# rll/rllab

Hardware: NVIDIA H100
Metric: env-steps/sec (full iteration: rollout + process_samples + VPG update) (higher is better)
Workload: dtype f32

## Files before the change

rllab_b200/csrc/update_umma32.cu:

```cuda
#include "tile_gram.cuh"
#include "umma_common.cuh"

namespace b200rl {

constexpr int V_THREADS = 128, V_TILE = 128, V_LD = V_TILE + 4;
#ifndef B200RL_V_PACKED_GRAM
#define B200RL_V_PACKED_GRAM 1
#endif

template <class N, int MODE>
struct Umma32 {
  static constexpr int O = N::O, H = 32, A = N::A;
  static_assert(N::H1 == 32 && N::H2 == 32 && O <= 24, "tensor-core 32-wide kernel: (32,32) nets, obs_dim <= 24");
  static constexpr int KX = ((O + 7) / 8) * 8;
  static constexpr int IMG = 32 * 32 * 4, IMGX = 32 * KX * 4;
  static constexpr int o_bXT = 0, o_bW1T = o_bXT + 2 * IMGX, o_bW1 = o_bW1T + 2 * IMG,
                       o_bV1T = o_bW1 + (MODE == MODE_LOSS ? 0 : 2 * IMG),
                       o_img_end = o_bV1T + (MODE == MODE_FVP ? 2 * IMG : 0);
  static constexpr int n_small = ((64 + 2 * H * A + A + 3) / 4) * 4;
  static constexpr int o_small = o_img_end, o_stage = o_small + n_small * 4;
  static constexpr int rX = 0, rH1 = rX + O, rH2 = rH1 + H, rD1 = rH2, rD2 = rH2 + H, rDM = rD2 + H, rDL = rDM + A,
                       R = (MODE == MODE_LOSS) ? 0 : rDL + A;
  static constexpr int RR = O + (MODE == MODE_FVP ? 0 : 2 * A + 1), qX = 0, qAct = O, qOm = O + A, qAdv = O + 2 * A;
  static constexpr int w_red = ((R * V_LD * 4 + 15) / 16) * 16, w_ring = w_red + 3 * 32 * 8,
                       w_bytes = w_ring + 2 * RR * V_LD * 4;
  static constexpr int o_wg = ((o_stage + 15) / 16) * 16;
  static_assert(MODE == MODE_LOSS || 2 * 64 * 16 * 8 <= R * V_LD * 4, "stage region must hold the K-half combine scratch");
  static constexpr int NWG = (MODE == MODE_LOSS || (is_grad_mode(MODE) && A == 1)) ? 3 : 2;
  static constexpr size_t bytes = (size_t)o_wg + (size_t)NWG * w_bytes;
  static_assert(bytes <= 232448, "does not fit the 227 KB of shared memory");
};

__device__ __forceinline__ void v_wg_sync(int wg) { asm volatile("bar.sync %0, 128;" ::"r"(wg + 1) : "memory"); }

template <int K, bool IS_MAX>
__device__ __forceinline__ void v_wg_reduce_store(const double (&v)[K], double* scratch, double* out, int tid, int wg) {
  const int lane = tid & 31, warp = tid >> 5;
#pragma unroll
  for (int k = 0; k < K; ++k) {
    double s = IS_MAX ? warp_max(v[k]) : warp_sum(v[k]);
    if (lane == 0) scratch[k * 32 + warp] = s;
  }
  v_wg_sync(wg);
  if (warp == 0) {
#pragma unroll
    for (int k = 0; k < K; ++k) {
      double s = lane < 4 ? scratch[k * 32 + lane] : (IS_MAX ? -1.0e300 : 0.0);
      s = IS_MAX ? warp_max(s) : warp_sum(s);
      if (lane == 0) out[k] = s;
    }
  }
  v_wg_sync(wg);
}

template <class SMT>
__device__ __forceinline__ void v_ring_load(const UpdArgs& a, float* ring, int slot, long long tile, int tid) {
  long long s = tile * V_TILE + tid;
  if (s >= a.B) s = a.B - 1;
  float* dst = ring + (size_t)slot * SMT::RR * V_LD + tid;
#pragma unroll
  for (int q = 0; q < SMT::RR; ++q) {
    const float* src = q < SMT::qAct ? a.obs + (size_t)q * a.B + s
                       : q < SMT::qOm ? a.act + (size_t)(q - SMT::qAct) * a.B + s
                       : q < SMT::qAdv ? a.old_mean + (size_t)(q - SMT::qOm) * a.B + s
                                       : a.adv + s;
    asm volatile("cp.async.ca.shared.global [%0], [%1], 4;" ::"r"(u_smem_u32(dst + q * V_LD)), "l"(src) : "memory");
  }
  asm volatile("cp.async.commit_group;" ::: "memory");
}

__device__ __forceinline__ int v_boff(int n, int k) {
  const int kp = u_kperm(k);
  return (kp & 3) * 4 + (n & 7) * 16 + (n >> 3) * 128 + (kp >> 2) * 512;
}

template <class N, int MODE>
__global__ void __launch_bounds__(V_THREADS * Umma32<N, MODE>::NWG, 1) update_umma32_kernel(UpdArgs a) {
  using SM = Umma32<N, MODE>;
  constexpr int O = N::O, H = 32, A = N::A, P = N::P, LD = V_LD, KX = SM::KX, KSX = KX / 8;
  extern __shared__ __align__(1024) unsigned char smem[];
  float* small = reinterpret_cast<float*>(smem + SM::o_small);
  float* sb0 = small, *sb1 = small + H, *sWout = small + 2 * H, *sVout = sWout + H * A;
  float* sbo = (MODE == MODE_FVP) ? sVout + H * A : sWout + H * A;
  constexpr int NWG = SM::NWG, NT = NWG * V_THREADS;
  const int gtid = threadIdx.x, wg = gtid >> 7, tid = gtid & (V_THREADS - 1), warp = tid >> 5, lane = tid & 31, t4 = lane & 3;
  unsigned char* wreg = smem + SM::o_wg + (size_t)wg * SM::w_bytes;
  float* stage = reinterpret_cast<float*>(wreg);
  double* red_scratch = reinterpret_cast<double*>(wreg + SM::w_red);
  float* ring = reinterpret_cast<float*>(wreg + SM::w_ring);

  for (int e = gtid; e < H * H; e += NT) {
    const int i = e / H, j = e % H;
    const float w = a.params[N::oW1 + e];
    const float wh = tf32_hi(w);
    *reinterpret_cast<float*>(smem + SM::o_bW1T + v_boff(j, i)) = wh;
    *reinterpret_cast<float*>(smem + SM::o_bW1T + SM::IMG + v_boff(j, i)) = w - wh;
    if constexpr (MODE != MODE_LOSS) {
      *reinterpret_cast<float*>(smem + SM::o_bW1 + v_boff(i, j)) = wh;
      *reinterpret_cast<float*>(smem + SM::o_bW1 + SM::IMG + v_boff(i, j)) = w - wh;
    }
    if constexpr (MODE == MODE_FVP) {
      const float v = (float)a.xvec[N::oW1 + e];
      const float vh = tf32_hi(v);
      *reinterpret_cast<float*>(smem + SM::o_bV1T + v_boff(j, i)) = vh;
      *reinterpret_cast<float*>(smem + SM::o_bV1T + SM::IMG + v_boff(j, i)) = v - vh;
    }
  }
  for (int e = gtid; e < KX * H; e += NT) {
    const int o = e / H, j = e % H;
    float v = 0.f;
    if (o < O) v = (MODE == MODE_FVP) ? (float)a.xvec[N::oW0 + o * H + j] : a.params[N::oW0 + o * H + j];
    const float vh = tf32_hi(v);
    *reinterpret_cast<float*>(smem + SM::o_bXT + v_boff(j, o)) = vh;
    *reinterpret_cast<float*>(smem + SM::o_bXT + SM::IMGX + v_boff(j, o)) = v - vh;
  }
  for (int e = gtid; e < H * A; e += NT) {
    sWout[e] = a.params[N::oWo + e];
    if constexpr (MODE == MODE_FVP) sVout[e] = (float)a.xvec[N::oWo + e];
  }
  for (int e = gtid; e < H; e += NT) {
    sb0[e] = (MODE == MODE_FVP) ? (float)a.xvec[N::ob0 + e] : a.params[N::ob0 + e];
    sb1[e] = (MODE == MODE_FVP) ? (float)a.xvec[N::ob1 + e] : a.params[N::ob1 + e];
  }
  if (gtid < A) sbo[gtid] = (MODE == MODE_FVP) ? (float)a.xvec[N::obo + gtid] : a.params[N::obo + gtid];
  asm volatile("fence.proxy.async.shared::cta;" ::: "memory");
  __syncthreads();

  TileDist D;
  tile_dist_init<N, MODE>(D, a.params + N::ols, a);

  const uint64_t dXT_hi = u_desc(u_smem_u32(smem + SM::o_bXT), 512, 128), dXT_lo = u_desc(u_smem_u32(smem + SM::o_bXT + SM::IMGX), 512, 128);
  const uint64_t dW1T_hi = u_desc(u_smem_u32(smem + SM::o_bW1T), 512, 128), dW1T_lo = u_desc(u_smem_u32(smem + SM::o_bW1T + SM::IMG), 512, 128);
  const uint64_t dW1_hi = u_desc(u_smem_u32(smem + SM::o_bW1), 512, 128), dW1_lo = u_desc(u_smem_u32(smem + SM::o_bW1 + SM::IMG), 512, 128);
  const uint64_t dV1T_hi = u_desc(u_smem_u32(smem + SM::o_bV1T), 512, 128), dV1T_lo = u_desc(u_smem_u32(smem + SM::o_bV1T + SM::IMG), 512, 128);

  auto gemm2 = [&](float (&acc)[2][16], auto& f, uint64_t b_hi, uint64_t b_lo, int KS, bool accumulate) {
    constexpr int NV = sizeof(f[0]) / sizeof(float);
#pragma unroll
    for (int mb = 0; mb < 2; ++mb) {
      uint32_t hi[NV], lo[NV];
      u_to_operand(f[mb], hi, lo);
      wg_split_gemm(acc[mb], hi, lo, b_hi, b_lo, 1024, KS, accumulate);
    }
  };

  TileGram<N, SM::rX, SM::rH1, SM::rH2, SM::rD1, SM::rD2, SM::rDM, LD, B200RL_V_PACKED_GRAM != 0> gram;
  if constexpr (MODE != MODE_LOSS) gram.init();
  double s_loss = 0.0, s_kl = 0.0, m_kl = -1.0e300;

  const int ntiles = (int)n_tiles_of(a, V_TILE), nvb = gridDim.x * NWG, vb = blockIdx.x * NWG + wg;
  if (vb < ntiles) v_ring_load<SM>(a, ring, 0, tile_at(a, vb), tid);
  int slot = 0;
  for (int ti_ = vb; ti_ < ntiles; ti_ += nvb, slot ^= 1) {
    const long long tile = tile_at(a, ti_);
    asm volatile("cp.async.wait_all;" ::: "memory");
    v_wg_sync(wg);
    if (ti_ + nvb < ntiles) v_ring_load<SM>(a, ring, slot ^ 1, tile_at(a, ti_ + nvb), tid);
    const float* rs = ring + (size_t)slot * SM::RR * V_LD;
    int trow[2][2];
    long long sl[2][2];
    bool inrange[2][2], valid[2][2];
#pragma unroll
    for (int mb = 0; mb < 2; ++mb)
#pragma unroll
      for (int h = 0; h < 2; ++h) {
        trow[mb][h] = mb * 64 + warp * 16 + u_frag_row(2 * h, lane);
        const long long s = tile * V_TILE + trow[mb][h];
        inrange[mb][h] = s < a.B;
        valid[mb][h] = sample_valid(a, s);
        sl[mb][h] = inrange[mb][h] ? s : a.B - 1;
      }
    float accA[2][16], accB[2][16];
    {
      float xf[2][4 * KSX];
#pragma unroll
      for (int mb = 0; mb < 2; ++mb)
#pragma unroll
        for (int i = 0; i < 4 * KSX; ++i) {
          const int o = u_frag_col(i, lane), h = (i >> 1) & 1;
          float x = 0.f;
          if (o < O) {
            x = rs[(SM::qX + o) * LD + trow[mb][h]];
            if constexpr (MODE != MODE_LOSS) stage[(SM::rX + o) * LD + trow[mb][h]] = x;
          }
          xf[mb][i] = x;
        }
      if constexpr (MODE == MODE_FVP) {
        float h1f[2][16];
#pragma unroll
        for (int mb = 0; mb < 2; ++mb)
#pragma unroll
          for (int i = 0; i < 16; ++i) {
            const int c = u_frag_col(i, lane), h = (i >> 1) & 1;
            h1f[mb][i] = a.h_cache[(size_t)c * a.B + sl[mb][h]];
            stage[(SM::rH1 + c) * LD + trow[mb][h]] = h1f[mb][i];
          }
        wg_fence();
        gemm2(accA, xf, dXT_hi, dXT_lo, KSX, false);
        gemm2(accB, h1f, dV1T_hi, dV1T_lo, 4, false);
        wg_commit();
      } else {
        wg_fence();
        gemm2(accA, xf, dXT_hi, dXT_lo, KSX, false);
        wg_commit();
      }
    }
    wg_wait_all();
#pragma unroll
    for (int mb = 0; mb < 2; ++mb) {
      wg_fence_operand(accA[mb]);
      wg_fence_operand(accB[mb]);
    }
    {
      float v[2][16];
#pragma unroll
      for (int mb = 0; mb < 2; ++mb)
#pragma unroll
        for (int i = 0; i < 16; ++i) {
          const int c = u_frag_col(i, lane), h = (i >> 1) & 1;
          if constexpr (MODE != MODE_FVP) {
            v[mb][i] = tanh_f(accA[mb][i] + sb0[c]);
            if constexpr (is_grad_mode(MODE)) {
              stage[(SM::rH1 + c) * LD + trow[mb][h]] = v[mb][i];
              if (a.h_cache != nullptr && inrange[mb][h]) a.h_cache[(size_t)c * a.B + sl[mb][h]] = v[mb][i];
            }
          } else {
            const float h1 = stage[(SM::rH1 + c) * LD + trow[mb][h]];
            v[mb][i] = (accA[mb][i] + sb0[c]) * (1.0f - h1 * h1);
          }
        }
      wg_fence();
      gemm2(accB, v, dW1T_hi, dW1T_lo, 4, MODE == MODE_FVP);
      wg_commit();
    }
    float h2f[2][16];
    if constexpr (MODE == MODE_FVP) {
#pragma unroll
      for (int mb = 0; mb < 2; ++mb)
#pragma unroll
        for (int i = 0; i < 16; ++i)
          h2f[mb][i] = a.h_cache[(size_t)(H + u_frag_col(i, lane)) * a.B + sl[mb][(i >> 1) & 1]];
    }
    wg_wait_all();
#pragma unroll
    for (int mb = 0; mb < 2; ++mb) wg_fence_operand(accB[mb]);
    {
      float md[2][2][A];
#pragma unroll
      for (int mb = 0; mb < 2; ++mb) {
#pragma unroll
        for (int h = 0; h < 2; ++h)
#pragma unroll
          for (int k = 0; k < A; ++k) md[mb][h][k] = 0.f;
#pragma unroll
        for (int i = 0; i < 16; ++i) {
          const int c = u_frag_col(i, lane), h = (i >> 1) & 1;
          if constexpr (MODE != MODE_FVP) {
            h2f[mb][i] = tanh_f(accB[mb][i] + sb1[c]);
            if constexpr (is_grad_mode(MODE)) {
              stage[(SM::rH2 + c) * LD + trow[mb][h]] = h2f[mb][i];
              if (a.h_cache != nullptr && inrange[mb][h]) a.h_cache[(size_t)(H + c) * a.B + sl[mb][h]] = h2f[mb][i];
            }
#pragma unroll
            for (int k = 0; k < A; ++k) md[mb][h][k] = fmaf(h2f[mb][i], sWout[c * A + k], md[mb][h][k]);
          } else {
            stage[(SM::rH2 + c) * LD + trow[mb][h]] = h2f[mb][i];
            const float t2 = (accB[mb][i] + sb1[c]) * (1.0f - h2f[mb][i] * h2f[mb][i]);
#pragma unroll
            for (int k = 0; k < A; ++k)
              md[mb][h][k] = fmaf(t2, sWout[c * A + k], fmaf(h2f[mb][i], sVout[c * A + k], md[mb][h][k]));
          }
        }
      }
#pragma unroll
      for (int mb = 0; mb < 2; ++mb)
#pragma unroll
        for (int h = 0; h < 2; ++h)
#pragma unroll
          for (int k = 0; k < A; ++k) {
            md[mb][h][k] += __shfl_xor_sync(0xffffffffu, md[mb][h][k], 1);
            md[mb][h][k] += __shfl_xor_sync(0xffffffffu, md[mb][h][k], 2);
          }
      float dmu[2][2][A];
#pragma unroll
      for (int mb = 0; mb < 2; ++mb)
#pragma unroll
        for (int h = 0; h < 2; ++h) {
          const int r = trow[mb][h];
          if constexpr (MODE != MODE_FVP) {
            float act[A], om[A];
#pragma unroll
            for (int k = 0; k < A; ++k) {
              act[k] = rs[(SM::qAct + k) * LD + r];
              om[k] = rs[(SM::qOm + k) * LD + r];
            }
            const float adv_s = rs[SM::qAdv * LD + r];
            float z[A], zz[A], dmk[A], zsq = 0.f, zsq_old = 0.f, kl = 0.f;
#pragma unroll
            for (int k = 0; k < A; ++k) {
              const float mu = sbo[k] + md[mb][h][k];
              z[k] = (act[k] - mu) * D.inv_std[k];
              zz[k] = __fmul_rn(z[k], z[k]);
              zsq += zz[k];
              const float zo = (act[k] - om[k]) * D.inv_std_old[k];
              zsq_old += zo * zo;
              const float dm = om[k] - mu;
              dmk[k] = dm;
              kl += (dm * dm + D.var_old[k] - D.var_new[k]) / D.var_new2[k] + D.ls_new[k] - D.ls_old[k];
            }
            const float logp_new = -D.sum_ls_new - 0.5f * zsq - D.half_log2pi_A;
            float w_s, term;
            if (a.loss_kind == B200RL_LOSS_TRPO) {
              const float logp_old = -D.sum_ls_old - 0.5f * zsq_old - D.half_log2pi_A;
              w_s = expf(logp_new - logp_old) * adv_s;
              term = -w_s;
            } else {
              w_s = adv_s;
              term = -logp_new * adv_s;
            }
            if (!valid[mb][h]) { w_s = 0.f; term = 0.f; }
            if (t4 == 0) {
              s_loss += (double)term;
              if (valid[mb][h]) { s_kl += (double)kl; m_kl = fmax(m_kl, (double)kl); }
            }
            if constexpr (is_grad_mode(MODE)) {
#pragma unroll
              for (int k = 0; k < A; ++k) {
                dmu[mb][h][k] = -w_s * z[k] * D.inv_std[k];
                if constexpr (MODE == MODE_GRAD_KL) {
                  float dls = -w_s * (zz[k] - 1.0f);
                  if (valid[mb][h])
                    add_kl_penalty(a.penalty, dmk[k], D.var_new[k], D.var_new2[k], D.var_old[k], dmu[mb][h][k], dls);
                  if (t4 == 0) {
                    stage[(SM::rDM + k) * LD + r] = dmu[mb][h][k];
                    stage[(SM::rDL + k) * LD + r] = dls;
                  }
                } else if (t4 == 0) {
                  stage[(SM::rDM + k) * LD + r] = dmu[mb][h][k];
                  stage[(SM::rDL + k) * LD + r] = -w_s * (zz[k] - 1.0f);
                }
              }
            }
          } else {
#pragma unroll
            for (int k = 0; k < A; ++k) {
              dmu[mb][h][k] = valid[mb][h] ? (sbo[k] + md[mb][h][k]) * D.Mmu[k] : 0.f;
              if (t4 == 0) {
                stage[(SM::rDM + k) * LD + r] = dmu[mb][h][k];
                stage[(SM::rDL + k) * LD + r] = 0.f;
              }
            }
          }
        }
      if constexpr (MODE != MODE_LOSS) {
        float v[2][16];
#pragma unroll
        for (int mb = 0; mb < 2; ++mb)
#pragma unroll
          for (int i = 0; i < 16; ++i) {
            const int c = u_frag_col(i, lane), h = (i >> 1) & 1;
            float sacc = 0.f;
#pragma unroll
            for (int k = 0; k < A; ++k) sacc = fmaf(dmu[mb][h][k], sWout[c * A + k], sacc);
            v[mb][i] = sacc * (1.0f - h2f[mb][i] * h2f[mb][i]);
            stage[(SM::rD2 + c) * LD + trow[mb][h]] = v[mb][i];
          }
        wg_fence();
        gemm2(accA, v, dW1_hi, dW1_lo, 4, false);
        wg_commit();
      }
    }
    if constexpr (MODE != MODE_LOSS) {
      constexpr bool wait_first = NWG >= 3;
      if constexpr (wait_first) {
        wg_wait_all();
#pragma unroll
        for (int mb = 0; mb < 2; ++mb) wg_fence_operand(accA[mb]);
      }
      v_wg_sync(wg);
      gram.accumulate_a(stage, tid);
      v_wg_sync(wg);
      if constexpr (!wait_first) {
        wg_wait_all();
#pragma unroll
        for (int mb = 0; mb < 2; ++mb) wg_fence_operand(accA[mb]);
      }
#pragma unroll
      for (int mb = 0; mb < 2; ++mb)
#pragma unroll
        for (int i = 0; i < 16; ++i) {
          const int c = u_frag_col(i, lane), r = trow[mb][(i >> 1) & 1];
          const float h1 = stage[(SM::rH1 + c) * LD + r];
          stage[(SM::rD1 + c) * LD + r] = accA[mb][i] * (1.0f - h1 * h1);
        }
      v_wg_sync(wg);
      gram.accumulate_b(stage, tid);
      v_wg_sync(wg);
    }
  }

  if constexpr (MODE != MODE_LOSS) {
    double* out = a.partial + (size_t)vb * P;
    gram.write(out, reinterpret_cast<double*>(stage), tid, [wg] { v_wg_sync(wg); });
  }
  if constexpr (MODE != MODE_FVP) {
    double v[2] = {s_loss, s_kl};
    double mx[1] = {m_kl};
    double* sc = a.partial + (is_grad_mode(MODE) ? (size_t)nvb * P : (size_t)0) + (size_t)vb * 3;
    v_wg_reduce_store<2, false>(v, red_scratch, sc, tid, wg);
    v_wg_reduce_store<1, true>(mx, red_scratch, sc + 2, tid, wg);
  }
}

template <class N, int MODE>
static int launch_umma32(const UpdArgs& a, int* grid_out, cudaStream_t st) {
  using SM = Umma32<N, MODE>;
  B200RL_SET_MAX_SMEM((update_umma32_kernel<N, MODE>), SM::bytes);
  long long grid = num_sms();
  const long long ntiles = host_n_tiles(a, V_TILE);
  if (grid > (ntiles + SM::NWG - 1) / SM::NWG) grid = (ntiles + SM::NWG - 1) / SM::NWG;
  if (grid > MAX_PARTIAL_BLOCKS / SM::NWG) grid = MAX_PARTIAL_BLOCKS / SM::NWG;
  if (grid < 1) grid = 1;
  update_umma32_kernel<N, MODE><<<(unsigned)grid, V_THREADS * SM::NWG, SM::bytes, st>>>(a);
  B200RL_LAUNCH_CHECK("update_umma32_kernel");
  *grid_out = (int)grid * SM::NWG;
  return 0;
}

int update_umma32_launch(int mode, int obs_dim, int act_dim, const UpdArgs& a, int* grid_out, int* P_out, int* ols_out,
                         cudaStream_t st) {
  const int h1 = 32, h2 = 32;
  B200RL_DISPATCH_NET_H(32, {
    *P_out = NetT::P;
    *ols_out = NetT::ols;
    int rc = (mode == MODE_GRAD)      ? launch_umma32<NetT, MODE_GRAD>(a, grid_out, st)
             : (mode == MODE_GRAD_KL) ? launch_umma32<NetT, MODE_GRAD_KL>(a, grid_out, st)
             : (mode == MODE_LOSS)    ? launch_umma32<NetT, MODE_LOSS>(a, grid_out, st)
                                      : launch_umma32<NetT, MODE_FVP>(a, grid_out, st);
    if (rc) return rc;
  });
  return 0;
}

}
```

Baseline: 2.058 billion.

## Process loss-mode tiles in 64-row halves and run more warpgroups per block

In loss-only mode the per-tile body now loops over the two 64-row halves one at a time (NB=1) instead of holding both in registers. This frees register and shared-memory budget so the block can run 4 to 6 warpgroups instead of 3, depending on action dim. The goal is more in-flight wgmma and latency hiding for the loss evaluation. The cost is serialised halves with extra wait/commit points per tile. Gradient and FVP modes keep NB=2 with the same structure.

```diff
diff --git a/rllab_b200/csrc/update_umma32.cu b/rllab_b200/csrc/update_umma32.cu
--- a/rllab_b200/csrc/update_umma32.cu
+++ b/rllab_b200/csrc/update_umma32.cu
@@ -26,7 +26,9 @@
                        w_bytes = w_ring + 2 * RR * V_LD * 4;
   static constexpr int o_wg = ((o_stage + 15) / 16) * 16;
   static_assert(MODE == MODE_LOSS || 2 * 64 * 16 * 8 <= R * V_LD * 4, "stage region must hold the K-half combine scratch");
-  static constexpr int NWG = (MODE == MODE_LOSS || (is_grad_mode(MODE) && A == 1)) ? 3 : 2;
+  static constexpr int NB = (MODE == MODE_LOSS) ? 1 : 2;
+  static constexpr int NWG = MODE == MODE_LOSS ? (A == 1 ? 6 : A <= 3 ? 5 : 4)
+                                               : (is_grad_mode(MODE) && A == 1) ? 3 : 2;
   static constexpr size_t bytes = (size_t)o_wg + (size_t)NWG * w_bytes;
   static_assert(bytes <= 232448, "does not fit the 227 KB of shared memory");
 };
@@ -82,7 +84,7 @@
   float* small = reinterpret_cast<float*>(smem + SM::o_small);
   float* sb0 = small, *sb1 = small + H, *sWout = small + 2 * H, *sVout = sWout + H * A;
   float* sbo = (MODE == MODE_FVP) ? sVout + H * A : sWout + H * A;
-  constexpr int NWG = SM::NWG, NT = NWG * V_THREADS;
+  constexpr int NWG = SM::NWG, NT = NWG * V_THREADS, NB = SM::NB;
   const int gtid = threadIdx.x, wg = gtid >> 7, tid = gtid & (V_THREADS - 1), warp = tid >> 5, lane = tid & 31, t4 = lane & 3;
   unsigned char* wreg = smem + SM::o_wg + (size_t)wg * SM::w_bytes;
   float* stage = reinterpret_cast<float*>(wreg);
@@ -134,10 +136,10 @@
   const uint64_t dW1_hi = u_desc(u_smem_u32(smem + SM::o_bW1), 512, 128), dW1_lo = u_desc(u_smem_u32(smem + SM::o_bW1 + SM::IMG), 512, 128);
   const uint64_t dV1T_hi = u_desc(u_smem_u32(smem + SM::o_bV1T), 512, 128), dV1T_lo = u_desc(u_smem_u32(smem + SM::o_bV1T + SM::IMG), 512, 128);
 
-  auto gemm2 = [&](float (&acc)[2][16], auto& f, uint64_t b_hi, uint64_t b_lo, int KS, bool accumulate) {
+  auto gemm2 = [&](float (&acc)[SM::NB][16], auto& f, uint64_t b_hi, uint64_t b_lo, int KS, bool accumulate) {
     constexpr int NV = sizeof(f[0]) / sizeof(float);
 #pragma unroll
-    for (int mb = 0; mb < 2; ++mb) {
+    for (int mb = 0; mb < NB; ++mb) {
       uint32_t hi[NV], lo[NV];
       u_to_operand(f[mb], hi, lo);
       wg_split_gemm(acc[mb], hi, lo, b_hi, b_lo, 1024, KS, accumulate);
@@ -157,245 +159,248 @@
     v_wg_sync(wg);
     if (ti_ + nvb < ntiles) v_ring_load<SM>(a, ring, slot ^ 1, tile_at(a, ti_ + nvb), tid);
     const float* rs = ring + (size_t)slot * SM::RR * V_LD;
-    int trow[2][2];
-    long long sl[2][2];
-    bool inrange[2][2], valid[2][2];
-#pragma unroll
-    for (int mb = 0; mb < 2; ++mb)
-#pragma unroll
-      for (int h = 0; h < 2; ++h) {
-        trow[mb][h] = mb * 64 + warp * 16 + u_frag_row(2 * h, lane);
-        const long long s = tile * V_TILE + trow[mb][h];
-        inrange[mb][h] = s < a.B;
-        valid[mb][h] = sample_valid(a, s);
-        sl[mb][h] = inrange[mb][h] ? s : a.B - 1;
-      }
-    float accA[2][16], accB[2][16];
-    {
-      float xf[2][4 * KSX];
-#pragma unroll
-      for (int mb = 0; mb < 2; ++mb)
-#pragma unroll
-        for (int i = 0; i < 4 * KSX; ++i) {
-          const int o = u_frag_col(i, lane), h = (i >> 1) & 1;
-          float x = 0.f;
-          if (o < O) {
-            x = rs[(SM::qX + o) * LD + trow[mb][h]];
-            if constexpr (MODE != MODE_LOSS) stage[(SM::rX + o) * LD + trow[mb][h]] = x;
+#pragma unroll 1
+    for (int mb0 = 0; mb0 < 2; mb0 += NB) {
+      int trow[NB][2];
+      long long sl[NB][2];
+      bool inrange[NB][2], valid[NB][2];
+#pragma unroll
+      for (int mb = 0; mb < NB; ++mb)
+#pragma unroll
+        for (int h = 0; h < 2; ++h) {
+          trow[mb][h] = (mb0 + mb) * 64 + warp * 16 + u_frag_row(2 * h, lane);
+          const long long s = tile * V_TILE + trow[mb][h];
+          inrange[mb][h] = s < a.B;
+          valid[mb][h] = sample_valid(a, s);
+          sl[mb][h] = inrange[mb][h] ? s : a.B - 1;
+        }
+      float accA[NB][16], accB[NB][16];
+      {
+        float xf[NB][4 * KSX];
+#pragma unroll
+        for (int mb = 0; mb < NB; ++mb)
+#pragma unroll
+          for (int i = 0; i < 4 * KSX; ++i) {
+            const int o = u_frag_col(i, lane), h = (i >> 1) & 1;
+            float x = 0.f;
+            if (o < O) {
+              x = rs[(SM::qX + o) * LD + trow[mb][h]];
+              if constexpr (MODE != MODE_LOSS) stage[(SM::rX + o) * LD + trow[mb][h]] = x;
+            }
+            xf[mb][i] = x;
           }
-          xf[mb][i] = x;
-        }
-      if constexpr (MODE == MODE_FVP) {
-        float h1f[2][16];
-#pragma unroll
-        for (int mb = 0; mb < 2; ++mb)
+        if constexpr (MODE == MODE_FVP) {
+          float h1f[NB][16];
+#pragma unroll
+          for (int mb = 0; mb < NB; ++mb)
+#pragma unroll
+            for (int i = 0; i < 16; ++i) {
+              const int c = u_frag_col(i, lane), h = (i >> 1) & 1;
+              h1f[mb][i] = a.h_cache[(size_t)c * a.B + sl[mb][h]];
+              stage[(SM::rH1 + c) * LD + trow[mb][h]] = h1f[mb][i];
+            }
+          wg_fence();
+          gemm2(accA, xf, dXT_hi, dXT_lo, KSX, false);
+          gemm2(accB, h1f, dV1T_hi, dV1T_lo, 4, false);
+          wg_commit();
+        } else {
+          wg_fence();
+          gemm2(accA, xf, dXT_hi, dXT_lo, KSX, false);
+          wg_commit();
+        }
+      }
+      wg_wait_all();
+#pragma unroll
+      for (int mb = 0; mb < NB; ++mb) {
+        wg_fence_operand(accA[mb]);
+        wg_fence_operand(accB[mb]);
+      }
+      {
+        float v[NB][16];
+#pragma unroll
+        for (int mb = 0; mb < NB; ++mb)
 #pragma unroll
           for (int i = 0; i < 16; ++i) {
             const int c = u_frag_col(i, lane), h = (i >> 1) & 1;
-            h1f[mb][i] = a.h_cache[(size_t)c * a.B + sl[mb][h]];
-            stage[(SM::rH1 + c) * LD + trow[mb][h]] = h1f[mb][i];
+            if constexpr (MODE != MODE_FVP) {
+              v[mb][i] = tanh_f(accA[mb][i] + sb0[c]);
+              if constexpr (is_grad_mode(MODE)) {
+                stage[(SM::rH1 + c) * LD + trow[mb][h]] = v[mb][i];
+                if (a.h_cache != nullptr && inrange[mb][h]) a.h_cache[(size_t)c * a.B + sl[mb][h]] = v[mb][i];
+              }
+            } else {
+              const float h1 = stage[(SM::rH1 + c) * LD + trow[mb][h]];
+              v[mb][i] = (accA[mb][i] + sb0[c]) * (1.0f - h1 * h1);
+            }
           }
         wg_fence();
-        gemm2(accA, xf, dXT_hi, dXT_lo, KSX, false);
-        gemm2(accB, h1f, dV1T_hi, dV1T_lo, 4, false);
+        gemm2(accB, v, dW1T_hi, dW1T_lo, 4, MODE == MODE_FVP);
         wg_commit();
-      } else {
-        wg_fence();
-        gemm2(accA, xf, dXT_hi, dXT_lo, KSX, false);
-        wg_commit();
-      }
-    }
-    wg_wait_all();
-#pragma unroll
-    for (int mb = 0; mb < 2; ++mb) {
-      wg_fence_operand(accA[mb]);
-      wg_fence_operand(accB[mb]);
-    }
-    {
-      float v[2][16];
-#pragma unroll
-      for (int mb = 0; mb < 2; ++mb)
-#pragma unroll
-        for (int i = 0; i < 16; ++i) {
-          const int c = u_frag_col(i, lane), h = (i >> 1) & 1;
-          if constexpr (MODE != MODE_FVP) {
-            v[mb][i] = tanh_f(accA[mb][i] + sb0[c]);
-            if constexpr (is_grad_mode(MODE)) {
-              stage[(SM::rH1 + c) * LD + trow[mb][h]] = v[mb][i];
-              if (a.h_cache != nullptr && inrange[mb][h]) a.h_cache[(size_t)c * a.B + sl[mb][h]] = v[mb][i];
-            }
-          } else {
-            const float h1 = stage[(SM::rH1 + c) * LD + trow[mb][h]];
-            v[mb][i] = (accA[mb][i] + sb0[c]) * (1.0f - h1 * h1);
-          }
-        }
-      wg_fence();
-      gemm2(accB, v, dW1T_hi, dW1T_lo, 4, MODE == MODE_FVP);
-      wg_commit();
-    }
-    float h2f[2][16];
-    if constexpr (MODE == MODE_FVP) {
-#pragma unroll
-      for (int mb = 0; mb < 2; ++mb)
-#pragma unroll
-        for (int i = 0; i < 16; ++i)
-          h2f[mb][i] = a.h_cache[(size_t)(H + u_frag_col(i, lane)) * a.B + sl[mb][(i >> 1) & 1]];
-    }
-    wg_wait_all();
-#pragma unroll
-    for (int mb = 0; mb < 2; ++mb) wg_fence_operand(accB[mb]);
-    {
-      float md[2][2][A];
-#pragma unroll
-      for (int mb = 0; mb < 2; ++mb) {
-#pragma unroll
-        for (int h = 0; h < 2; ++h)
-#pragma unroll
-          for (int k = 0; k < A; ++k) md[mb][h][k] = 0.f;
-#pragma unroll
-        for (int i = 0; i < 16; ++i) {
-          const int c = u_frag_col(i, lane), h = (i >> 1) & 1;
-          if constexpr (MODE != MODE_FVP) {
-            h2f[mb][i] = tanh_f(accB[mb][i] + sb1[c]);
-            if constexpr (is_grad_mode(MODE)) {
-              stage[(SM::rH2 + c) * LD + trow[mb][h]] = h2f[mb][i];
-              if (a.h_cache != nullptr && inrange[mb][h]) a.h_cache[(size_t)(H + c) * a.B + sl[mb][h]] = h2f[mb][i];
-            }
-#pragma unroll
-            for (int k = 0; k < A; ++k) md[mb][h][k] = fmaf(h2f[mb][i], sWout[c * A + k], md[mb][h][k]);
-          } else {
-            stage[(SM::rH2 + c) * LD + trow[mb][h]] = h2f[mb][i];
-            const float t2 = (accB[mb][i] + sb1[c]) * (1.0f - h2f[mb][i] * h2f[mb][i]);
-#pragma unroll
-            for (int k = 0; k < A; ++k)
-              md[mb][h][k] = fmaf(t2, sWout[c * A + k], fmaf(h2f[mb][i], sVout[c * A + k], md[mb][h][k]));
-          }
-        }
-      }
-#pragma unroll
-      for (int mb = 0; mb < 2; ++mb)
-#pragma unroll
-        for (int h = 0; h < 2; ++h)
-#pragma unroll
-          for (int k = 0; k < A; ++k) {
-            md[mb][h][k] += __shfl_xor_sync(0xffffffffu, md[mb][h][k], 1);
-            md[mb][h][k] += __shfl_xor_sync(0xffffffffu, md[mb][h][k], 2);
-          }
-      float dmu[2][2][A];
-#pragma unroll
-      for (int mb = 0; mb < 2; ++mb)
-#pragma unroll
-        for (int h = 0; h < 2; ++h) {
-          const int r = trow[mb][h];
-          if constexpr (MODE != MODE_FVP) {
-            float act[A], om[A];
-#pragma unroll
-            for (int k = 0; k < A; ++k) {
-              act[k] = rs[(SM::qAct + k) * LD + r];
-              om[k] = rs[(SM::qOm + k) * LD + r];
-            }
-            const float adv_s = rs[SM::qAdv * LD + r];
-            float z[A], zz[A], dmk[A], zsq = 0.f, zsq_old = 0.f, kl = 0.f;
-#pragma unroll
-            for (int k = 0; k < A; ++k) {
-              const float mu = sbo[k] + md[mb][h][k];
-              z[k] = (act[k] - mu) * D.inv_std[k];
-              zz[k] = __fmul_rn(z[k], z[k]);
-              zsq += zz[k];
-              const float zo = (act[k] - om[k]) * D.inv_std_old[k];
-              zsq_old += zo * zo;
-              const float dm = om[k] - mu;
-              dmk[k] = dm;
-              kl += (dm * dm + D.var_old[k] - D.var_new[k]) / D.var_new2[k] + D.ls_new[k] - D.ls_old[k];
-            }
-            const float logp_new = -D.sum_ls_new - 0.5f * zsq - D.half_log2pi_A;
-            float w_s, term;
-            if (a.loss_kind == B200RL_LOSS_TRPO) {
-              const float logp_old = -D.sum_ls_old - 0.5f * zsq_old - D.half_log2pi_A;
-              w_s = expf(logp_new - logp_old) * adv_s;
-              term = -w_s;
-            } else {
-              w_s = adv_s;
-              term = -logp_new * adv_s;
-            }
-            if (!valid[mb][h]) { w_s = 0.f; term = 0.f; }
-            if (t4 == 0) {
-              s_loss += (double)term;
-              if (valid[mb][h]) { s_kl += (double)kl; m_kl = fmax(m_kl, (double)kl); }
-            }
-            if constexpr (is_grad_mode(MODE)) {
-#pragma unroll
-              for (int k = 0; k < A; ++k) {
-                dmu[mb][h][k] = -w_s * z[k] * D.inv_std[k];
-                if constexpr (MODE == MODE_GRAD_KL) {
-                  float dls = -w_s * (zz[k] - 1.0f);
-                  if (valid[mb][h])
-                    add_kl_penalty(a.penalty, dmk[k], D.var_new[k], D.var_new2[k], D.var_old[k], dmu[mb][h][k], dls);
-                  if (t4 == 0) {
-                    stage[(SM::rDM + k) * LD + r] = dmu[mb][h][k];
-                    stage[(SM::rDL + k) * LD + r] = dls;
-                  }
-                } else if (t4 == 0) {
-                  stage[(SM::rDM + k) * LD + r] = dmu[mb][h][k];
-                  stage[(SM::rDL + k) * LD + r] = -w_s * (zz[k] - 1.0f);
-                }
-              }
-            }
-          } else {
-#pragma unroll
-            for (int k = 0; k < A; ++k) {
-              dmu[mb][h][k] = valid[mb][h] ? (sbo[k] + md[mb][h][k]) * D.Mmu[k] : 0.f;
-              if (t4 == 0) {
-                stage[(SM::rDM + k) * LD + r] = dmu[mb][h][k];
-                stage[(SM::rDL + k) * LD + r] = 0.f;
-              }
-            }
-          }
-        }
-      if constexpr (MODE != MODE_LOSS) {
-        float v[2][16];
-#pragma unroll
-        for (int mb = 0; mb < 2; ++mb)
+      }
+      float h2f[NB][16];
+      if constexpr (MODE == MODE_FVP) {
+#pragma unroll
+        for (int mb = 0; mb < NB; ++mb)
+#pragma unroll
+          for (int i = 0; i < 16; ++i)
+            h2f[mb][i] = a.h_cache[(size_t)(H + u_frag_col(i, lane)) * a.B + sl[mb][(i >> 1) & 1]];
+      }
+      wg_wait_all();
+#pragma unroll
+      for (int mb = 0; mb < NB; ++mb) wg_fence_operand(accB[mb]);
+      {
+        float md[NB][2][A];
+#pragma unroll
+        for (int mb = 0; mb < NB; ++mb) {
+#pragma unroll
+          for (int h = 0; h < 2; ++h)
+#pragma unroll
+            for (int k = 0; k < A; ++k) md[mb][h][k] = 0.f;
 #pragma unroll
           for (int i = 0; i < 16; ++i) {
             const int c = u_frag_col(i, lane), h = (i >> 1) & 1;
-            float sacc = 0.f;
-#pragma unroll
-            for (int k = 0; k < A; ++k) sacc = fmaf(dmu[mb][h][k], sWout[c * A + k], sacc);
-            v[mb][i] = sacc * (1.0f - h2f[mb][i] * h2f[mb][i]);
-            stage[(SM::rD2 + c) * LD + trow[mb][h]] = v[mb][i];
+            if constexpr (MODE != MODE_FVP) {
+              h2f[mb][i] = tanh_f(accB[mb][i] + sb1[c]);
+              if constexpr (is_grad_mode(MODE)) {
+                stage[(SM::rH2 + c) * LD + trow[mb][h]] = h2f[mb][i];
+                if (a.h_cache != nullptr && inrange[mb][h]) a.h_cache[(size_t)(H + c) * a.B + sl[mb][h]] = h2f[mb][i];
+              }
+#pragma unroll
+              for (int k = 0; k < A; ++k) md[mb][h][k] = fmaf(h2f[mb][i], sWout[c * A + k], md[mb][h][k]);
+            } else {
+              stage[(SM::rH2 + c) * LD + trow[mb][h]] = h2f[mb][i];
+              const float t2 = (accB[mb][i] + sb1[c]) * (1.0f - h2f[mb][i] * h2f[mb][i]);
+#pragma unroll
+              for (int k = 0; k < A; ++k)
+                md[mb][h][k] = fmaf(t2, sWout[c * A + k], fmaf(h2f[mb][i], sVout[c * A + k], md[mb][h][k]));
+            }
           }
-        wg_fence();
-        gemm2(accA, v, dW1_hi, dW1_lo, 4, false);
-        wg_commit();
-      }
-    }
-    if constexpr (MODE != MODE_LOSS) {
-      constexpr bool wait_first = NWG >= 3;
-      if constexpr (wait_first) {
-        wg_wait_all();
-#pragma unroll
-        for (int mb = 0; mb < 2; ++mb) wg_fence_operand(accA[mb]);
-      }
-      v_wg_sync(wg);
-      gram.accumulate_a(stage, tid);
-      v_wg_sync(wg);
-      if constexpr (!wait_first) {
-        wg_wait_all();
-#pragma unroll
-        for (int mb = 0; mb < 2; ++mb) wg_fence_operand(accA[mb]);
-      }
-#pragma unroll
-      for (int mb = 0; mb < 2; ++mb)
-#pragma unroll
-        for (int i = 0; i < 16; ++i) {
-          const int c = u_frag_col(i, lane), r = trow[mb][(i >> 1) & 1];
-          const float h1 = stage[(SM::rH1 + c) * LD + r];
-          stage[(SM::rD1 + c) * LD + r] = accA[mb][i] * (1.0f - h1 * h1);
-        }
-      v_wg_sync(wg);
-      gram.accumulate_b(stage, tid);
-      v_wg_sync(wg);
+        }
+#pragma unroll
+        for (int mb = 0; mb < NB; ++mb)
+#pragma unroll
+          for (int h = 0; h < 2; ++h)
+#pragma unroll
+            for (int k = 0; k < A; ++k) {
+              md[mb][h][k] += __shfl_xor_sync(0xffffffffu, md[mb][h][k], 1);
+              md[mb][h][k] += __shfl_xor_sync(0xffffffffu, md[mb][h][k], 2);
+            }
+        float dmu[NB][2][A];
+#pragma unroll
+        for (int mb = 0; mb < NB; ++mb)
+#pragma unroll
+          for (int h = 0; h < 2; ++h) {
+            const int r = trow[mb][h];
+            if constexpr (MODE != MODE_FVP) {
+              float act[A], om[A];
+#pragma unroll
+              for (int k = 0; k < A; ++k) {
+                act[k] = rs[(SM::qAct + k) * LD + r];
+                om[k] = rs[(SM::qOm + k) * LD + r];
+              }
+              const float adv_s = rs[SM::qAdv * LD + r];
+              float z[A], zz[A], dmk[A], zsq = 0.f, zsq_old = 0.f, kl = 0.f;
+#pragma unroll
+              for (int k = 0; k < A; ++k) {
+                const float mu = sbo[k] + md[mb][h][k];
+                z[k] = (act[k] - mu) * D.inv_std[k];
+                zz[k] = __fmul_rn(z[k], z[k]);
+                zsq += zz[k];
+                const float zo = (act[k] - om[k]) * D.inv_std_old[k];
+                zsq_old += zo * zo;
+                const float dm = om[k] - mu;
+                dmk[k] = dm;
+                kl += (dm * dm + D.var_old[k] - D.var_new[k]) / D.var_new2[k] + D.ls_new[k] - D.ls_old[k];
+              }
+              const float logp_new = -D.sum_ls_new - 0.5f * zsq - D.half_log2pi_A;
+              float w_s, term;
+              if (a.loss_kind == B200RL_LOSS_TRPO) {
+                const float logp_old = -D.sum_ls_old - 0.5f * zsq_old - D.half_log2pi_A;
+                w_s = expf(logp_new - logp_old) * adv_s;
+                term = -w_s;
+              } else {
+                w_s = adv_s;
+                term = -logp_new * adv_s;
+              }
+              if (!valid[mb][h]) { w_s = 0.f; term = 0.f; }
+              if (t4 == 0) {
+                s_loss += (double)term;
+                if (valid[mb][h]) { s_kl += (double)kl; m_kl = fmax(m_kl, (double)kl); }
+              }
+              if constexpr (is_grad_mode(MODE)) {
+#pragma unroll
+                for (int k = 0; k < A; ++k) {
+                  dmu[mb][h][k] = -w_s * z[k] * D.inv_std[k];
+                  if constexpr (MODE == MODE_GRAD_KL) {
+                    float dls = -w_s * (zz[k] - 1.0f);
+                    if (valid[mb][h])
+                      add_kl_penalty(a.penalty, dmk[k], D.var_new[k], D.var_new2[k], D.var_old[k], dmu[mb][h][k], dls);
+                    if (t4 == 0) {
+                      stage[(SM::rDM + k) * LD + r] = dmu[mb][h][k];
+                      stage[(SM::rDL + k) * LD + r] = dls;
+                    }
+                  } else if (t4 == 0) {
+                    stage[(SM::rDM + k) * LD + r] = dmu[mb][h][k];
+                    stage[(SM::rDL + k) * LD + r] = -w_s * (zz[k] - 1.0f);
+                  }
+                }
+              }
+            } else {
+#pragma unroll
+              for (int k = 0; k < A; ++k) {
+                dmu[mb][h][k] = valid[mb][h] ? (sbo[k] + md[mb][h][k]) * D.Mmu[k] : 0.f;
+                if (t4 == 0) {
+                  stage[(SM::rDM + k) * LD + r] = dmu[mb][h][k];
+                  stage[(SM::rDL + k) * LD + r] = 0.f;
+                }
+              }
+            }
+          }
+        if constexpr (MODE != MODE_LOSS) {
+          float v[NB][16];
+#pragma unroll
+          for (int mb = 0; mb < NB; ++mb)
+#pragma unroll
+            for (int i = 0; i < 16; ++i) {
+              const int c = u_frag_col(i, lane), h = (i >> 1) & 1;
+              float sacc = 0.f;
+#pragma unroll
+              for (int k = 0; k < A; ++k) sacc = fmaf(dmu[mb][h][k], sWout[c * A + k], sacc);
+              v[mb][i] = sacc * (1.0f - h2f[mb][i] * h2f[mb][i]);
+              stage[(SM::rD2 + c) * LD + trow[mb][h]] = v[mb][i];
+            }
+          wg_fence();
+          gemm2(accA, v, dW1_hi, dW1_lo, 4, false);
+          wg_commit();
+        }
+      }
+      if constexpr (MODE != MODE_LOSS) {
+        constexpr bool wait_first = NWG >= 3;
+        if constexpr (wait_first) {
+          wg_wait_all();
+#pragma unroll
+          for (int mb = 0; mb < NB; ++mb) wg_fence_operand(accA[mb]);
+        }
+        v_wg_sync(wg);
+        gram.accumulate_a(stage, tid);
+        v_wg_sync(wg);
+        if constexpr (!wait_first) {
+          wg_wait_all();
+#pragma unroll
+          for (int mb = 0; mb < NB; ++mb) wg_fence_operand(accA[mb]);
+        }
+#pragma unroll
+        for (int mb = 0; mb < NB; ++mb)
+#pragma unroll
+          for (int i = 0; i < 16; ++i) {
+            const int c = u_frag_col(i, lane), r = trow[mb][(i >> 1) & 1];
+            const float h1 = stage[(SM::rH1 + c) * LD + r];
+            stage[(SM::rD1 + c) * LD + r] = accA[mb][i] * (1.0f - h1 * h1);
+          }
+        v_wg_sync(wg);
+        gram.accumulate_b(stage, tid);
+        v_wg_sync(wg);
+      }
     }
   }
 
```

New measurement: 2.105 billion (median of 6 runs). +2.3%, better.
